# mrcdr/lambda-lanczos

Measured on AMD Instinct MI355X. Metric: Lanczos iterations/sec + SpMV GB/s (fp64, n=10M nnz=150M) at 1/2/4/8 GPUs, higher is better.
Workload: dtype f64; 1 GPU; random symmetric CSR n=10000000 nnz=150000000 fp64; n=10000000, nnz=150000000, partition=single GPU, orth_mode=0, tridiag_mode=2, eps=engine default

## Files before the change

### lambda-lanczos_amd/csrc/context.cpp

```cpp
#include <algorithm>
#include <cstdlib>
#include <memory>

#include "engine.hpp"

namespace ll {
static thread_local std::string g_last_error;
void set_error(const std::string& msg) { g_last_error = msg; }
}

using namespace ll;

namespace ll {
namespace {
long long to_ll(const std::string& v) { return std::atoll(v.c_str()); }
bool to_flag(const std::string& v) { return std::atoi(v.c_str()) != 0; }
int Tuning::*pauli_bits_key(const std::string& key) {
  static const std::pair<const char*, int Tuning::*> keys[] = {
      {"pauli_tile_bits", &Tuning::pauli_tile_bits}, {"pauli_sector_block_bits", &Tuning::pauli_sector_block_bits},
      {"pauli_momentum_block_bits", &Tuning::pauli_momentum_block_bits},
      {"pauli_momentum_full_block_bits", &Tuning::pauli_momentum_full_block_bits},
      {"pauli_symmetric_block_bits", &Tuning::pauli_symmetric_block_bits},
      {"pauli_rdm_tile_bits", &Tuning::pauli_rdm_tile_bits}, {"pauli_rdm_block_bits", &Tuning::pauli_rdm_block_bits}};
  for (const auto& k : keys)
// ... 17 lines not shown
  else if (key == "pair_gs") t.pair_gs = e ? d.pair_gs : to_flag(v);
  else if (key == "block_gs") t.block_gs = e ? d.block_gs : to_flag(v);
  else if (key == "pb_diag") t.pb_diag = e ? d.pb_diag : to_flag(v);
  else if (key == "fuse_launches") {
    const long long level = e ? 2 : to_ll(v);
    t.fuse_launches = level >= 1;
    t.lagged_gs = level >= 2;
  } else if (key == "blas_small_bytes") t.blas_small_bytes = e ? d.blas_small_bytes : to_ll(v);
  else if (key == "tridiag_thread") t.tridiag_thread = e ? d.tridiag_thread : to_flag(v);
  else if (key == "tridiag_lag") t.tridiag_lag = e ? d.tridiag_lag : (int)to_ll(v);
  else if (key == "dgks_threshold") t.dgks_threshold = e ? d.dgks_threshold : std::atof(v.c_str());
  else if (key == "slab_bytes") t.slab_bytes = e ? d.slab_bytes : std::max<long long>(1, to_ll(v));
  else if (key == "pb_block") t.pb_block = e ? 0 : (int)std::max<long long>(0, to_ll(v));
  else if (key == "pb_row_block") t.pb_row_block = e ? 0 : (int)std::max<long long>(0, to_ll(v));
  else if (key == "pb_col_block") t.pb_col_block = e ? 0 : (int)std::max<long long>(0, to_ll(v));
  else if (key == "pb_threads1") {
    t.pb_threads1 = e ? 0 : (int)to_ll(v);
    if (t.pb_threads1 != 256 && t.pb_threads1 != 512 && t.pb_threads1 != 1024) t.pb_threads1 = 0;
  } else if (key == "pb_pad") {
    t.pb_pad = e ? 0 : (int)to_ll(v);
    if (t.pb_pad != 4 && t.pb_pad != 16) t.pb_pad = 0;
  } else if (key == "pb_xpre") t.pb_xpre = e ? d.pb_xpre : to_flag(v);
  else if (key == "pb_test_all_remote") t.pb_test_all_remote = e ? false : to_flag(v);
  else if (key == "force_rp64") t.force_rp64 = e ? false : to_flag(v);
  else if (key == "spmv_tile_balance") t.spmv_tile_balance = e ? d.spmv_tile_balance : to_flag(v);
  else if (int Tuning::*bits = pauli_bits_key(key)) t.*bits = e ? d.*bits : (int)std::max<long long>(0, std::min<long long>(30, to_ll(v)));
  else if (key == "stencil_vec") t.stencil_vec = e ? d.stencil_vec : to_flag(v);
  else if (key == "tl_force") t.tl_force = e ? false : to_flag(v);
  else if (key == "tl_xcd") t.tl_xcd_order = e ? d.tl_xcd_order : to_flag(v);
  else if (key == "tl_walk") t.tl_walk_modulo = e ? d.tl_walk_modulo : to_flag(v);
  else if (key == "ritz_tail") t.ritz_tail = e ? d.ritz_tail : to_flag(v);
  else if (key == "event_in_launch") t.event_in_launch = e ? d.event_in_launch : to_flag(v);
  else if (key == "sweep_pipeline") t.sweep_pipeline = e ? d.sweep_pipeline : (int)std::max<long long>(0, std::min<long long>(2, to_ll(v)));
  else if (key == "pair_split") t.pair_split_vecs = e ? 0 : (int)std::max<long long>(0, to_ll(v));
  else if (key == "pair_max_stored") t.pair_max_stored = e ? 0 : (int)std::max<long long>(0, to_ll(v));
  else if (key == "lagged_pieces") t.lagged_pieces = e ? 0 : (int)to_ll(v);
  else if (key == "lagged_min_bytes") t.lagged_min_bytes = e ? -1 : to_ll(v);
  else if (key == "tridiag_test_jitter_us") t.tridiag_test_jitter_us = e ? 0 : (int)to_ll(v);
  else if (key == "test_workspace_fill") t.test_workspace_fill = e ? -1 : (int)std::max<long long>(0, std::min<long long>(255, to_ll(v)));
  else if (key == "stall_trace") t.stall_trace_ms = e ? -1.0 : std::atof(v.c_str());
  else return false;
  return true;
}
static const char* const kEnvSwitches[][2] = {
    {"LL_SPMV_KERNEL", "spmv_kernel"},       {"LL_SPMV_KEEP_BOTH", "spmv_keep_both"}, {"LL_PB_PHASE2", "pb_phase2"},
    {"LL_PB_PLACEMENTS", "pb_placements"},   {"LL_PB_PLACEMENT_TRACE", "pb_placement_trace"},
    {"LL_COMM_OVERLAP", "comm_overlap"},     {"LL_GATHER_CHUNKS", "gather_chunks"},   {"LL_CSR_SPLIT", "csr_split"},
    {"LL_ITER_TRACE", "iter_trace"},         {"LL_SHARDED_NORM", "sharded_norm"},     {"LL_PAIR_GS", "pair_gs"},
    {"LL_PB_DIAG", "pb_diag"},               {"LL_FUSE_LAUNCHES", "fuse_launches"},   {"LL_BLAS_SMALL_BYTES", "blas_small_bytes"},
    {"LL_TRIDIAG_THREAD", "tridiag_thread"}, {"LL_TRIDIAG_LAG", "tridiag_lag"},       {"LL_DGKS_THRESHOLD", "dgks_threshold"},
    {"LL_SLAB_BYTES", "slab_bytes"},
};
Tuning read_tuning(const std::map<std::string, std::string>* overrides) {
  Tuning t;
  for (auto& sw : kEnvSwitches) {
    const char* e = std::getenv(sw[0]);
    if (e && *e) (void)tuning_apply(t, sw[1], e);
  }
  if (overrides)
    for (auto& kv : *overrides) (void)tuning_apply(t, kv.first, kv.second);
  return t;
}
}

static size_t grow(size_t have, size_t want) { return std::max(want, have + have / 2 + 64); }

// ... 436 lines not shown
```

### lambda-lanczos_amd/csrc/gs_block.hip

```cpp
#include <algorithm>

#include "gs_strips.hpp"

namespace ll {

namespace {
__device__ __forceinline__ void block_sum2_all(double& a, double& b, double* sh) {
  a = wave_sum(a);
  b = wave_sum(b);
  const int lane = threadIdx.x & 63, wave = threadIdx.x >> 6;
  __syncthreads();
  if (lane == 0) {
    sh[wave] = a;
    sh[4 + wave] = b;
  }
  __syncthreads();
  a = (sh[0] + sh[1]) + (sh[2] + sh[3]);
  b = (sh[4] + sh[5]) + (sh[6] + sh[7]);
}
__device__ __forceinline__ void block_max2_all(double& a, double& b, double* sh) {
#pragma unroll
  for (int d = 32; d > 0; d >>= 1) {
    a = fmax(a, __shfl_down(a, d, 64));
    b = fmax(b, __shfl_down(b, d, 64));
// ... 4 lines not shown
    sh[wave] = a;
    sh[4 + wave] = b;
  }
  __syncthreads();
  a = fmax(fmax(sh[0], sh[1]), fmax(sh[2], sh[3]));
  b = fmax(fmax(sh[4], sh[5]), fmax(sh[6], sh[7]));
}
__device__ __forceinline__ double block_tri_row(const double* __restrict__ ha, const double* __restrict__ hb, const double* v, int i,
                                                int reals, int m, double alpha_last) {
  const int j = i / reals;
  double t = (j == m - 1 ? alpha_last : ha[j]) * v[i];
  if (j >= 1) t = fma(hb[j - 1], v[i - reals], t);
  if (j + 1 < m) t = fma(hb[j], v[i + reals], t);
  return t;
}
__device__ __forceinline__ size_t block_row_at(int reals, int j) { return (size_t)reals * (size_t)j * (size_t)(j - 1) / 2; }
}

__global__ __launch_bounds__(256) void block_enter_kernel(int k, int reals, const double* __restrict__ g, const double* __restrict__ c1,
                                                          double* __restrict__ rho2, double* __restrict__ cpk) {
  const int tid = threadIdx.x;
  for (int j = tid; j < k; j += 256) rho2[j] = 1.0;
  if (tid == 0) rho2[k] = *c1;
  double* rk1 = cpk + block_row_at(reals, k - 1);
  for (int i = tid; i < reals * (k - 1); i += 256) rk1[i] = 0.0;
  double* rk = cpk + block_row_at(reals, k);
  for (int i = tid; i < reals * k; i += 256) rk[i] = g[i];
}
void launch_block_enter(int k, int reals, const double* g, const double* c1, double* rho2, double* cpk, hipStream_t s) {
  hipLaunchKernelGGL(block_enter_kernel, dim3(1), dim3(256), 0, s, k, reals, g, c1, rho2, cpk);
  LL_HIP(hipGetLastError());
}

__global__ __launch_bounds__(256) void block_predict_kernel(int k, int m, int reals, BlockScalars sc, const double* __restrict__ rho2,
                                                            const double* __restrict__ cpk, double* __restrict__ hist_alpha,
                                                            const double* __restrict__ hist_beta, double* __restrict__ dk,
                                                            double* __restrict__ p, int pstride, double* __restrict__ prA,
                                                            double* __restrict__ prB) {
  __shared__ double red[8];
  const int tid = threadIdx.x;
  const int W = k + 1, RW = reals * W;
  const double* ck = cpk + block_row_at(reals, k);
  const double* ck1 = cpk + block_row_at(reals, k - 1);
  const double rk = sqrt(rho2[k]), rk1 = sqrt(rho2[k - 1]);
  const double ik = 1.0 / rk, ik1 = 1.0 / rk1;
  const double e0 = *sc.e[0];
  for (int i = tid; i < RW; i += 256) dk[i] = i < reals * k ? ck[i] * ik : 0.0;
  __syncthreads();
  double qa = 0.0, zero_ = 0.0;
  for (int i = tid; i < reals * k; i += 256) qa = fma(dk[i], block_tri_row(hist_alpha, hist_beta, dk, i, reals, k, hist_alpha[k - 1]), qa);
  block_sum2_all(qa, zero_, red);
  const double ake = -2.0 * ck[reals * (k - 1)] - qa;
  const double alpha_k = e0 + ake;
  if (tid == 0) hist_alpha[k] = alpha_k;
  for (int i = tid; i < RW; i += 256) {
    const double t = block_tri_row(hist_alpha, hist_beta, dk, i, reals, W, alpha_k);
    const double d1 = i < reals * (k - 1) ? ck1[i] * ik1 : 0.0;
    double v = t - e0 * dk[i] - rk * d1;
    if (i == reals * k) v += ake;
    p[i] = v;
  }
  __syncthreads();
  for (int s = 1; s < m; ++s) {
    const double* in = p + (size_t)(s - 1) * pstride;
    const double nin = sqrt(*sc.nsq[s - 1]), inv = 1.0 / nin;
    const double* prev = s == 1 ? dk : p + (size_t)(s - 2) * pstride;
    const double pinv = s == 1 ? 1.0 : 1.0 / sqrt(*sc.nsq[s - 2]);
    const double es = *sc.e[s];
    double* out = p + (size_t)s * pstride;
    for (int i = tid; i < RW; i += 256) {
      const double t = block_tri_row(hist_alpha, hist_beta, in, i, reals, W, alpha_k);
      out[i] = (t - es * in[i]) * inv - nin * (prev[i] * pinv);
    }
    __syncthreads();
  }
  for (int i = tid; i < RW; i += 256) {
    const double ir = 1.0 / sqrt(rho2[i / reals]);
    prA[i] = p[(size_t)(m - 1) * pstride + i] * ir;
    prB[i] = m >= 2 ? p[(size_t)(m - 2) * pstride + i] * ir : 0.0;
  }
}
void launch_block_predict(int k, int m, int reals, const BlockScalars& sc, const double* rho2, const double* cpk, double* hist_alpha,
                          const double* hist_beta, double* dk, double* p, int pstride, double* prA, double* prB, hipStream_t s) {
  hipLaunchKernelGGL(block_predict_kernel, dim3(1), dim3(256), 0, s, k, m, reals, sc, rho2, cpk, hist_alpha, hist_beta, dk, p, pstride, prA,
                     prB);
  LL_HIP(hipGetLastError());
}

template <typename T, int NV, int PC, int M>
__device__ __forceinline__ void block_trip_compute(const T (&ur)[NV][strip<T, PC>::EPT], int nv, const T (&b)[M][strip<T, PC>::EPT],
                                                   T (&cA)[strip<T, PC>::EPT], T (&cB)[strip<T, PC>::EPT],
                                                   const double* __restrict__ prAc, const double* __restrict__ prBc, double* mine,
                                                   int setstride, int lane) {
  constexpr int EPT = strip<T, PC>::EPT;
  double sre[M][NV], sim[M][NV];
#pragma unroll
  for (int v = 0; v < NV; ++v) {
    acc_t<T> ca, cb;
    const int vv = v < nv ? v : nv - 1;
    const bool real = v < nv;
    if constexpr (scalar_traits<T>::is_complex) {
      const double xa = ld_const(prAc, 2 * vv), ya = ld_const(prAc, 2 * vv + 1), xb = ld_const(prBc, 2 * vv), yb = ld_const(prBc, 2 * vv + 1);
      ca = zc{real ? xa : 0.0, real ? ya : 0.0};
      cb = zc{real ? xb : 0.0, real ? yb : 0.0};
    } else {
      const double xa = ld_const(prAc, vv), xb = ld_const(prBc, vv);
      ca = real ? xa : 0.0;
      cb = real ? xb : 0.0;
    }
    acc_t<T> sm[M];
#pragma unroll
    for (int i = 0; i < M; ++i) sm[i] = zero<acc_t<T>>();
#pragma unroll
    for (int e = 0; e < EPT; ++e) {
      fnma_acc(cA[e], ca, ur[v][e]);
      if constexpr (M >= 2) fnma_acc(cB[e], cb, ur[v][e]);
#pragma unroll
      for (int i = 0; i < M; ++i) cfma_acc(sm[i], ur[v][e], b[i][e]);
    }
#pragma unroll
    for (int i = 0; i < M; ++i) {
      if constexpr (scalar_traits<T>::is_complex) {
        sre[i][v] = sm[i].re;
        sim[i][v] = sm[i].im;
      } else {
        sre[i][v] = sm[i];
        sim[i][v] = 0.0;
      }
    }
  }
  constexpr int LPI = 64 / NV;
#pragma unroll
  for (int i = 0; i < M; ++i) {
    wave_sum_transposed<NV>(sre[i], lane);
    if constexpr (scalar_traits<T>::is_complex) wave_sum_transposed<NV>(sim[i], lane);
  }
  if ((lane & (LPI - 1)) == 0 && lane / LPI < nv) {
    const int v = lane / LPI;
#pragma unroll
    for (int i = 0; i < M; ++i) {
      if constexpr (scalar_traits<T>::is_complex) {
        mine[i * setstride + 2 * v] += sre[i][0];
        mine[i * setstride + 2 * v + 1] += sim[i][0];
      } else {
        mine[i * setstride + v] += sre[i][0];
      }
    }
  }
}

template <typename T, int PC, int M, int JB>
__global__ __launch_bounds__(kBlock) void block_sweep_kernel(int64_t n, const T* const* __restrict__ vtab, int W, int col0, int Wl, int flags,
                                                             BlockVecs<T> bv, const double* __restrict__ prA,
                                                             const double* __restrict__ prB, double* __restrict__ partials) {
  constexpr int EPT = strip<T, PC>::EPT;
  constexpr int ELEMS = strip<T, PC>::ELEMS;
  constexpr int R = scalar_traits<T>::reals;
  constexpr int NG = R * M * (M - 1) / 2 + M;
  const bool first = (flags & kPairFirst) != 0, last = (flags & kPairLast) != 0;
  const int ncols = M * R * W + NG;
  const int lcols = M * R * Wl + (last ? NG : 0);
  extern __shared__ double lds[];
  const int tid = threadIdx.x, lane = tid & 63, wave = tid >> 6;
  for (int i = tid; i < 4 * lcols; i += kBlock) lds[i] = 0.0;
  __syncthreads();
  double* mine = lds + (size_t)wave * lcols;
  double* tail = mine + M * R * Wl;
  const T* const* tab = vtab + col0;
  const double *prAc = prA + R * col0, *prBc = prB + R * col0;
  const int ntrips = (Wl + JB - 1) / JB;
  const int64_t nstrips = (n + ELEMS - 1) / ELEMS;
  T* const outA = last ? bv.b[M - 1] : bv.part[0];
  T* const outB = last ? bv.b[M >= 2 ? M - 2 : 0] : bv.part[1];

  auto do_strip = [&](auto full_c, const int64_t base) {
    constexpr bool FULL = decltype(full_c)::value;
    T b[M][EPT], cA[EPT], cB[EPT];
#pragma unroll
    for (int i = 0; i < M; ++i) load_lstrip_u<T, PC, FULL>(bv.b[i], base, n, b[i]);
    auto issue = [&](T (&buf)[JB][EPT], int t) {
      const T* ptr[JB];
#pragma unroll
      for (int v = 0; v < JB; ++v) ptr[v] = ld_const_ptr<T>(tab, min(JB * t + v, Wl - 1));
#pragma unroll
      for (int v = 0; v < JB; ++v) load_lstrip_u<T, PC, FULL>(ptr[v], base, n, buf[v]);
    };
    T ua[JB][EPT], ub[JB][EPT];
    if (ntrips > 0) {
      __builtin_amdgcn_sched_barrier(0);
      issue(ua, 0);
      __builtin_amdgcn_sched_barrier(0);
    }
    if (first) {
#pragma unroll
      for (int e = 0; e < EPT; ++e) {
        cA[e] = b[M - 1][e];
        cB[e] = b[M >= 2 ? M - 2 : 0][e];
      }
    } else {
      load_lstrip_u<T, PC, FULL>(bv.part[0], base, n, cA);
      if constexpr (M >= 2) load_lstrip_u<T, PC, FULL>(bv.part[1], base, n, cB);
    }
    for (int t = 0; t < ntrips; t += 2) {
      __builtin_amdgcn_sched_barrier(0);
      issue(ub, t + 1);
      __builtin_amdgcn_sched_barrier(0);
      block_trip_compute<T, JB, PC, M>(ua, min(JB, Wl - JB * t), b, cA, cB, prAc + R * JB * t, prBc + R * JB * t, mine + R * JB * t, R * Wl, lane);
      if (t + 1 >= ntrips) break;
      __builtin_amdgcn_sched_barrier(0);
      issue(ua, t + 2);
      __builtin_amdgcn_sched_barrier(0);
      block_trip_compute<T, JB, PC, M>(ub, min(JB, Wl - JB * (t + 1)), b, cA, cB, prAc + R * JB * (t + 1), prBc + R * JB * (t + 1),
                                       mine + R * JB * (t + 1), R * Wl, lane);
    }
    store_lstrip_u<T, PC, FULL>(outA, base, n, cA);
    if constexpr (M >= 2) store_lstrip_u<T, PC, FULL>(outB, base, n, cB);
    if (!last) return;
#pragma unroll
    for (int e = 0; e < EPT; ++e) {
      b[M - 1][e] = cA[e];
      if constexpr (M >= 2) b[M - 2][e] = cB[e];
    }
    int at = 0;
#pragma unroll
    for (int i = 1; i < M; ++i) {
#pragma unroll
      for (int ip = 0; ip < i; ++ip) {
        acc_t<T> g = zero<acc_t<T>>();
#pragma unroll
        for (int e = 0; e < EPT; ++e) cfma_acc(g, b[ip][e], b[i][e]);
        const acc_t<T> gs = wave_sum(g);
        if (lane == 0) {
          if constexpr (scalar_traits<T>::is_complex) {
            tail[at] += gs.re;
            tail[at + 1] += gs.im;
          } else {
            tail[at] += gs;
          }
        }
        at += R;
      }
    }
#pragma unroll
    for (int i = 0; i < M; ++i) {
      double nn = 0.0;
#pragma unroll
      for (int e = 0; e < EPT; ++e) nn += abs2(b[i][e]);
      nn = wave_sum(nn);
      if (lane == 0) tail[at + i] += nn;
    }
  };
  for (int64_t sidx = blockIdx.x; sidx < nstrips; sidx += gridDim.x) {
    const int64_t base = sidx * ELEMS;
    if (base + ELEMS <= n) do_strip(std::true_type{}, base);
    else do_strip(std::false_type{}, base);
  }
  __syncthreads();
  double* out = partials + (size_t)blockIdx.x * ncols;
  for (int i = tid; i < lcols; i += kBlock) {
    const double v = (lds[i] + lds[lcols + i]) + (lds[2 * lcols + i] + lds[3 * lcols + i]);
    int g;
    if (i < M * R * Wl) {
      const int set = i / (R * Wl);
      g = set * R * W + R * col0 + (i - set * R * Wl);
    } else {
      g = M * R * W + (i - M * R * Wl);
    }
    out[g] = v;
  }
}
constexpr int kBlockJB = 2;
template <typename T, int PC, int M>
static void block_sweep_launch(int grid, size_t lds_bytes, hipStream_t s, int64_t n, const T* const* vtab, int W, int col0, int Wl, int flags,
                               const BlockVecs<T>& bv, const double* prA, const double* prB, double* partials) {
  hipLaunchKernelGGL((block_sweep_kernel<T, PC, M, kBlockJB>), dim3(grid), dim3(kBlock), lds_bytes, s, n, vtab, W, col0, Wl, flags, bv, prA, prB,
                     partials);
}
template <typename T>
int launch_block_sweep(int64_t n, const T* const* vtab, int W, int m, const BlockVecs<T>& bv, const double* prA, const double* prB,
                       double* partials, int pieces, int per_launch, hipStream_t s) {
  constexpr int R = scalar_traits<T>::reals;
  LL_REQUIRE(m == 1 || m == 2 || m == 4, "internal: block sweep of 1, 2 or 4 iterations");
  const int64_t strips16k = (n * (int64_t)sizeof(T) + 16383) / 16384;
  int pc = strips16k >= kLaggedFullStrips ? 4 : 2;
  if (pieces == 2 || pieces == 4) pc = pieces;
  const int grid = pc == 4 ? strip_grid(n, strip<T, 4>::ELEMS) : strip_grid(n, strip<T, 2>::ELEMS);
  const int ng = R * m * (m - 1) / 2 + m;
  per_launch = std::max(1, std::min(per_launch, block_sweep_max_vecs<T>(m)));
  for (int col0 = 0; col0 < W; col0 += per_launch) {
    const int Wl = std::min(per_launch, W - col0);
    const int flags = (col0 == 0 ? kPairFirst : 0) | (col0 + Wl == W ? kPairLast : 0);
    const size_t lds_bytes = (size_t)4 * (size_t)(m * R * Wl + ((flags & kPairLast) ? ng : 0)) * sizeof(double);
#define LL_BLOCK_SWEEP(PC_, M_) block_sweep_launch<T, PC_, M_>(grid, lds_bytes, s, n, vtab, W, col0, Wl, flags, bv, prA, prB, partials)
    if (pc == 4) {
      if (m == 4) LL_BLOCK_SWEEP(4, 4);
      else if (m == 2) LL_BLOCK_SWEEP(4, 2);
      else LL_BLOCK_SWEEP(4, 1);
    } else {
      if (m == 4) LL_BLOCK_SWEEP(2, 4);
      else if (m == 2) LL_BLOCK_SWEEP(2, 2);
      else LL_BLOCK_SWEEP(2, 1);
    }
#undef LL_BLOCK_SWEEP
    LL_HIP(hipGetLastError());
  }
  return grid;
}

__global__ __launch_bounds__(256) void block_fold_kernel(const double* __restrict__ cols, int k, int m, int reals, BlockScalars sc,
                                                         const double* __restrict__ p, int pstride, double* __restrict__ rho2,
                                                         double* __restrict__ cpk, double* __restrict__ hist_alpha,
                                                         double* __restrict__ hist_beta, double* __restrict__ raw0,
                                                         double* __restrict__ raw1, BlockHost host) {
  __shared__ double red[8];
  const int tid = threadIdx.x;
  const int W = k + 1, RW = reals * W;
  const double* tail = cols + (size_t)m * RW;
  const double* diag = tail + reals * m * (m - 1) / 2;
  for (int s = 0; s < m; ++s) {
    const int j = k + 1 + s;
    double* raw = (s & 1) ? raw1 : raw0;
    const double* rawp = (s & 1) ? raw0 : raw1;
    double* row = cpk + block_row_at(reals, j);
    const double* ms = cols + (size_t)s * RW;
    const double* ps = p + (size_t)s * pstride;
    const bool comp = s == m - 1 || s == m - 2;
    const double nn = diag[s], nraw2 = *sc.nsq[s];
    for (int i = tid; i < RW; i += 256) raw[i] = ms[i] / sqrt(rho2[i / reals]);
    __syncthreads();
    for (int col = k - 1; col <= k; ++col) {
      const double* cr = cpk + block_row_at(reals, col);
      double dre = 0.0, dim = 0.0;
      for (int l = tid; l < col; l += 256) {
        if (reals == 2) {
          const double ar = cr[2 * l], ai = cr[2 * l + 1], br = raw[2 * l], bi = raw[2 * l + 1];
          dre += ar * br + ai * bi;
          dim += ar * bi - ai * br;
        } else {
          dre += cr[l] * raw[l];
        }
      }
      block_sum2_all(dre, dim, red);
      if (tid == 0) {
        const double ir = 1.0 / sqrt(rho2[col]);
        raw[reals * col] = (ms[reals * col] - dre) * ir;
        if (reals == 2) raw[2 * col + 1] = (ms[2 * col + 1] - dim) * ir;
      }
      __syncthreads();
    }
    double mxr = 0.0, mxc = 0.0, cc = 0.0;
    for (int i = tid; i < RW; i += 256) {
      const double v = comp ? raw[i] - ps[i] : raw[i];
      row[i] = v;
      mxr = fmax(mxr, fabs(raw[i]));
      mxc = fmax(mxc, fabs(v));
      cc = fma(v, v, cc);
    }
    __syncthreads();
    for (int sp = 0; sp < s; ++sp) {
      const int col = k + 1 + sp;
// ... 28 lines not shown
    }
    double zero_ = 0.0;
    block_sum2_all(cc, zero_, red);
    block_max2_all(mxr, mxc, red);
    double r2 = nn - cc;
    r2 = r2 > 0.0 ? r2 : 0.0;
    double alpha_pub;
    if (s == 0) {
      alpha_pub = hist_alpha[k];
    } else {
      double qb = 0.0;
      for (int i = tid; i < reals * (j - 1); i += 256)
        qb = fma(rawp[i], block_tri_row(hist_alpha, hist_beta, rawp, i, reals, j - 1, hist_alpha[j - 2]), qb);
      block_sum2_all(qb, zero_, red);
      const double rp2 = rho2[j - 1];
      alpha_pub = rp2 > 0.0 ? (*sc.e[s] * *sc.nsq[s - 1] - 2.0 * rp2 * rawp[reals * (j - 2)] - qb) / rp2 : 0.0;
    }
    __syncthreads();
    if (tid == 0) {
      rho2[j] = r2;
      hist_beta[j - 1] = sqrt(r2);
      if (s > 0) hist_alpha[j - 1] = alpha_pub;
      double gate = 1.0;
      if (nn > 0.0 && nraw2 > 0.0) gate = fmax(mxr / sqrt(nraw2), mxc / sqrt(nn));
      host.slot[s][0] = alpha_pub;
      host.slot[s][1] = r2;
      host.slot[s][2] = nn;
      host.slot[s][3] = r2;
      *host.gate[s] = gate;
    }
    __syncthreads();
  }
}
void launch_block_fold(const double* cols, int k, int m, int reals, const BlockScalars& sc, const double* p, int pstride, double* rho2,
                       double* cpk, double* hist_alpha, double* hist_beta, double* raw0, double* raw1, const BlockHost& host, hipStream_t s,
                       hipEvent_t stop) {
  LL_LAUNCH_STOP(stop, block_fold_kernel, dim3(1), dim3(256), 0, s, cols, k, m, reals, sc, p, pstride, rho2, cpk, hist_alpha, hist_beta, raw0,
                 raw1, host);
  LL_HIP(hipGetLastError());
}

template int launch_block_sweep<double>(int64_t, const double* const*, int, int, const BlockVecs<double>&, const double*, const double*,
                                        double*, int, int, hipStream_t);
template int launch_block_sweep<zc>(int64_t, const zc* const*, int, int, const BlockVecs<zc>&, const double*, const double*, double*, int, int,
                                    hipStream_t);

}
```

### lambda-lanczos_amd/csrc/lanczos_loop.hpp

```cpp
#pragma once

#include "engine.hpp"
#include "loop_support.hpp"
#include "raw_basis.hpp"
#include "ritz_tracker.hpp"
#include "trace.hpp"

#include <algorithm>
#include <cmath>
#include <limits>
#include <string>
#include <variant>

namespace ll {


template <typename T> struct LoopState {
  Engine<T>& E;
  Basis<T>& U;
  EventRing& ring;
  PhaseTimer& timer;
  int64_t nl;
  hipStream_t s;
  bool fuse_launches = true, defer = false;
// ... 382 lines not shown
    coeff = pair_coeff_over_raw(R, g1h, g2h, std::sqrt(rho[0]), std::sqrt(rho[1]), n_locked, Pt, tail.nvec, m, nw, coeff);
    basis = basis_runs(Pt);
    basis.add(tail.pair.r[0], 1);
    if (tail.nvec == 2) basis.add(tail.pair.r[1], 1);
    return basis;
  }
  int64_t enqueue_block(int64_t kk, double offset) {
    if constexpr (sizeof(typename scalar_traits<T>::real) == 8) return enqueue_block_f64(kk, offset);
    else return 0;
  }
  int64_t enqueue_block_f64(int64_t kk, double offset) {
    constexpr int R = Engine<T>::R;
    const Tuning& tune = E.ctx->tune;
    if (!block_enabled || !block_allowed || !pair_allowed || !lag_ok || n_locked != 0) return 0;
    const BlockIter* const bi = pending_as<BlockIter>();
    const LaggedIter* const lg = pending_as<LaggedIter>();
    int64_t k;
    if (bi) {
      if (bi->k + 1 != kk) return 0;
      k = bi->k;
    } else if (lg && lg->k == kk - 1 && kk >= 3) {
      k = kk - 1;
    } else {
      return 0;
    }
    const int64_t remaining = max_k_hint - (kk - 1);
    if (remaining < 1) return 0;
    const int m = remaining >= 4 ? 4 : (remaining >= 2 ? 2 : 1);
    const int64_t strips16k = (nl * (int64_t)sizeof(T) + 16383) / 16384;
    const bool streaming = tune.sweep_pipeline >= 2 || strips16k > 2 * kCUs + kCUs / 4;
    if (!streaming || vec_bytes() < stream_bytes() || k + m + 1 > bb.cap || (size_t)(k + m + 1) > kVtabCap) return 0;
    if (tune.pair_max_stored > 0 && k + 1 > tune.pair_max_stored) return 0;
    const int W = (int)(k + 1);
    const int ncols = m * R * W + R * m * (m - 1) / 2 + m;
    int per_launch = block_sweep_max_vecs<T>(m);
    if (tune.pair_split_vecs > 0) per_launch = std::min(per_launch, std::max(1, tune.pair_split_vecs));
    if (W > per_launch)
      for (auto& b : bsplit)
        if (!b.p) b.alloc(E.ctx, (size_t)ld);
    const double te0 = now_s();
    want_partial_cols((size_t)std::max(ncols, 1 + R));
    if (!bi) {
      LL_HIP(hipMemcpyAsync(U.vec(k), work[k & 1].p, (size_t)nl * sizeof(T), hipMemcpyDeviceToDevice, s));
      launch_block_enter((int)k, R, lb.g[k & 1], lg->c1, bb.rho2, bb.cpk, s);
      blk_k0 = k;
    }
    BlockVecs<T> bv{};
    for (int i = 0; i < m; ++i) bv.b[i] = U.vec(k + 1 + i);
    bv.part[0] = bsplit[0].p;
    bv.part[1] = bsplit[1].p;
    const T* const* vt = vtab_sync();
    BlockScalars sc{};
    BlockHost host{};
    int slots[4] = {0, 0, 0, 0};
    for (int i = 0; i < 4; ++i) {
      const int ii = std::min(i, m - 1);
      slots[i] = (int)((kk + ii) % kRingSlots);
      sc.e[i] = E.S(kScalAlpha + slots[i]);
      sc.nsq[i] = bb.nsq + 4 * ii;
      host.slot[i] = pinned_slot(slots[i]);
      host.gate[i] = pinned_gate(slots[i]);
    }
    for (int i = 0; i < m; ++i) {
      const T* x = i == 0 ? U.vec(k) : bv.b[i - 1];
      const T* xp = i == 0 ? U.vec(k - 1) : (i == 1 ? U.vec(k) : bv.b[i - 2]);
      const double* xn2 = i == 0 ? bb.rho2 + k : bb.nsq + 4 * (i - 1);
      const double* pn2 = i == 0 ? bb.rho2 + k - 1 : (i == 1 ? bb.rho2 + k : bb.nsq + 4 * (i - 2));
      double* e = E.S(kScalAlpha + slots[i]);
      timer.mark();
      typename Engine<T>::DeferredAlpha da;
      E.apply(x, bv.b[i], offset, e, true, fuse_launches ? &da : nullptr, nullptr, xn2);
      timer.mark();
      const int g3 = launch_pair_three_term<T>(nl, bv.b[i], x, xp, e, da.nparts > 0 ? da.partials : nullptr, da.nparts, xn2, pn2,
                                               E.ctx->partials.get(), false, s);
      launch_reduce_cols(E.ctx->partials.get(), g3, 1 + R, bb.nsq + 4 * i, nullptr, s);
      if (i + 1 < m) timer.mark();
    }
    launch_block_predict((int)k, m, R, sc, bb.rho2, bb.cpk, lb.hist_alpha, lb.hist_beta, bb.dk, bb.p, (int)bb.rec, bb.prA, bb.prB, s);
    const int grid = launch_block_sweep<T>(nl, vt, W, m, bv, bb.prA, bb.prB, E.ctx->partials.get(), tune.lagged_pieces, per_launch, s);
    launch_reduce_cols(E.ctx->partials.get(), grid, ncols, bb.cols, nullptr, s);
    const int ev = slots[m - 1];
    launch_block_fold(bb.cols, (int)k, m, R, sc, bb.p, (int)bb.rec, bb.rho2, bb.cpk, lb.hist_alpha, lb.hist_beta, bb.raw0, bb.raw1, host, s,
                      tune.event_in_launch ? ring.ev[ev] : nullptr);
    if (!tune.event_in_launch) LL_HIP(hipEventRecord(ring.ev[ev], s));
    timer.mark();
    for (int i = 0; i < m; ++i) {
      ev_of_slot[slots[i]] = ev;
      slot_pair[slots[i]] = true;
    }
    pending = BlockIter{k + m};
    n_block += m;
    if (m >= 2) n_pair += m;
    n_lagged += m;
    t_enqueue += now_s() - te0;
    return m;
  }
  bool enqueue_pair(int64_t k, double offset) {
    constexpr int R = Engine<T>::R;
    if (!pair_enabled || !pair_allowed || !lag_ok) return false;
    if (max_k_hint > 0 && k + 1 > max_k_hint) return false;
    const int64_t Lk = n_locked;
    PairIter in;
    if (const PairIter* pr = pending_as<PairIter>()) {
      if (pr->P + 2 != k) return false;
      in = *pr;
    } else if (const LaggedIter* lg = pending_as<LaggedIter>(); lg && lg->k == k - 1 && k >= 3) {
      in = PairIter{k - 2, {U.vec(k - 2), work[(k - 1) & 1].p}, {pb.zero, lb.g[(k - 1) & 1]}, {pb.scal + 0, lg->c1}, 0, 1};
    } else {
      return false;
    }
    const int64_t P = in.P;
    const T *const r1 = in.r[0], *const r2 = in.r[1];
    const double *const g1 = in.g[0], *const g2 = in.g[1], *const rho1sq = in.rho2[0], *const rho2sq = in.rho2[1];
    const int out_set = in.set ^ 1, out_rec = in.rec ^ 1;
    const int64_t K = Lk + P;
// ... 354 lines not shown
```

### lambda-lanczos_amd/csrc/ll_internal.hpp

```cpp
#pragma once

#include <hip/hip_runtime.h>
#if defined(__HIPCC__)
#include <hip/hip_ext.h>
#endif

#include <algorithm>
#include <atomic>
#include <cstdint>
#include <cstdio>
#include <cstring>
#include <map>
#include <memory>
#include <string>
#include <type_traits>
#include <vector>

#include "../../include/lanczos_hip.h"
#include "../../include/lanczos_hip_transport.h"
#include "scalar_types.hpp"
#include "spmv_plan.hpp"

#if defined(__HIPCC__)
#define LL_LAUNCH_STOP(stop, kernel, grid, block, lds, s, ...)                                      \
// ... 151 lines not shown
namespace ll {
struct Tuning {
  int spmv_kernel = -1;
  bool keep_both = false;
  int pb_phase2 = 4;
  int pb_block = 0;
  int pb_row_block = 0;
  int pb_col_block = 0;
  int pair_max_stored = 0;
  int pair_split_vecs = 0;
  int pb_threads1 = 0;
  int pb_pad = 0;
  int pb_placements = 8;
  bool pb_xpre = true;
  bool pb_diag = true;
  int gather_chunks = 0;
  bool spmv_tile_balance = true;
  bool csr_split = true;
  bool comm_overlap = true;
  bool tridiag_thread = true;
  int tridiag_lag = 3;
  double dgks_threshold = 0.5;
  bool sharded_norm_measured = false;
  int64_t slab_bytes = (int64_t)4 << 30;
  int64_t blas_small_bytes = (int64_t)4 << 20;
  bool fuse_launches = true;
  long long lagged_min_bytes = -1;
  int lagged_pieces = 0;
  bool lagged_gs = true;
  bool event_in_launch = true;
  bool ritz_tail = true;
  int sweep_pipeline = 1;
  bool block_gs = true;
  bool pair_gs = true;
  bool force_rp64 = false;
  bool tl_xcd_order = true;
  bool tl_walk_modulo = true;
  bool tl_force = false;
  bool pb_test_all_remote = false;
  int tridiag_test_jitter_us = 0;
  int pauli_tile_bits = -1;
  int pauli_momentum_block_bits = -1;
  int pauli_momentum_full_block_bits = -1;
  int pauli_symmetric_block_bits = -1;
  int pauli_sector_block_bits = -1;
  int pauli_rdm_tile_bits = -1;
  int pauli_rdm_block_bits = -1;
  int test_workspace_fill = -1;
  bool stencil_vec = true;
  double stall_trace_ms = -1.0;
  std::string iter_trace;
  bool pb_placement_trace = false;
};
Tuning read_tuning(const std::map<std::string, std::string>* overrides);
bool tuning_apply(Tuning& t, const std::string& key, const std::string& value);

}

struct ll_context {
  ll::Tuning tune;
  std::map<std::string, std::string> tuning_overrides;
  int device = 0;
  hipStream_t stream = nullptr;
  bool own_stream = false;
  ll::Comm* comm = nullptr;
  int rank = 0, nranks = 1;
// ... 427 lines not shown
template <typename T> constexpr int pair_sweep_max_vecs() {
  return (kLaggedMaxCols - 5 * scalar_traits<T>::reals - 1) / (2 * scalar_traits<T>::reals);
}
template <typename T>
int launch_pair_sweep(int64_t n, const std::vector<BasisSegs<T>>& groups, int P, const T* r1, const T* r2, const T* r3, T* r4,
                      T* uP_out, T* uQ_out, T* part4, const double* g1, const double* g2, const double* gam, const double* p4,
                      const double* rho1sq, const double* rho2sq, const double* e2, const double* n3sq, double* partials, int pieces,
                      hipStream_t s, const T* const* vtab = nullptr,
                      bool force_pipeline = false);
template <typename T>
bool launch_pair_sweep_small(int64_t n, const BasisSegs<T>& segs, int P, const T* r1, const T* r2, const T* r3, T* r4, T* uP_out,
                             T* uQ_out, const double* g1, const double* g2, const double* gam, const double* p4, const double* rho1sq,
                             const double* rho2sq, const double* e2, const double* n3sq, double* partials, int* grid_out,
                             hipStream_t s);
template <typename T> bool pair_small_fits(int P);
template <typename T> void launch_fill_ptrs(const T** tab, int start, int count, const T* base, int64_t ld, hipStream_t s);
void launch_pair_fold(const double* m, int P, int L, int reals, const double* lambda, const double* p4, const double* g2, const double* gam,
                      const double* rho2sq, const double* n3sq, const double* e1, const double* e2, double* rec3, double* rec4,
                      double* nxt, double* hist_alpha, double* hist_beta, double* scratch, double* host_a, double* host_b,
                      double* gate_a, double* gate_b, hipStream_t s, hipEvent_t stop = nullptr);
constexpr int kBlockMaxVecs = 1024;
struct BlockScalars {
  const double* e[4];
  const double* nsq[4];
};
struct BlockHost {
  double* slot[4];
  double* gate[4];
};
template <typename T> struct BlockVecs {
  T* b[4];
  T* part[2];
};
template <typename T> constexpr int block_sweep_max_vecs(int m) {
  return (kLaggedMaxCols - (scalar_traits<T>::reals * m * (m - 1) / 2 + m)) / (m * scalar_traits<T>::reals);
}
void launch_block_enter(int k, int reals, const double* g, const double* c1, double* rho2, double* cpk, hipStream_t s);
void launch_block_predict(int k, int m, int reals, const BlockScalars& sc, const double* rho2, const double* cpk, double* hist_alpha,
                          const double* hist_beta, double* dk, double* p, int pstride, double* prA, double* prB, hipStream_t s);
template <typename T>
int launch_block_sweep(int64_t n, const T* const* vtab, int W, int m, const BlockVecs<T>& bv, const double* prA, const double* prB,
                       double* partials, int pieces, int per_launch, hipStream_t s);
void launch_block_fold(const double* cols, int k, int m, int reals, const BlockScalars& sc, const double* p, int pstride, double* rho2,
                       double* cpk, double* hist_alpha, double* hist_beta, double* raw0, double* raw1, const BlockHost& host, hipStream_t s,
                       hipEvent_t stop = nullptr);
void launch_lagged_fold(double* m, int K, int L, int reals, double* t_out, const double* c0, double* c0_out, double* c1,
                        double* alpha, const double* prev_g, const double* prev_t, const double* prev_c1,
                        double* hist_alpha, double* hist_beta, const double* lambda, double* host_mapped, hipStream_t s, hipEvent_t stop = nullptr);
template <typename T>
int launch_maxpy(int64_t n, T* w, const BasisSegs<T>& segs, const double* h, const NormRefs* pred, double* partials,
                 int64_t small_bytes, hipStream_t s);
template <typename T>
bool launch_maxpy_folding(int64_t n, T* w, const BasisSegs<T>& segs, const double* mdot_partials, int mparts, double* h_out,
                          double* c0_out, double* partials, int64_t small_bytes, int* grid_out, hipStream_t s);
template <typename T> void launch_scale(int64_t n, T* v, double a, const NormRefs* norms, hipStream_t s);
template <typename T>
void launch_scale_derive(int64_t n, T* v, const double* c0_src, const double* h, int count, double* c0, double* c1,
                         const double* alpha, double* host_mapped, hipStream_t s);
template <typename T>
int launch_scale_publish(int64_t n, T* v, const double* partials, int nparts, double* out, const double* alpha,
                         const double* c0, double* host_mapped, hipStream_t s, const T* src = nullptr);
template <typename T>
void launch_three_term(int64_t n, T* w, const T* u_prev, const T* u_cur, double beta, double alpha, hipStream_t s);
constexpr int kRecurRec = 4;
template <typename T>
int launch_recur_step(int64_t n, T* y, const T* x, const T* p, const double* alpha_partials, int alpha_nparts, double* rec,
                      int64_t k, bool normalised, double* partials, hipStream_t s);
void launch_recur_fold(const double* partials, int nparts, double* rec, int64_t k, double* host_mapped, hipStream_t s);
template <typename T>
void launch_recur_accum(int64_t n, T* y, const T* x, const T* p, T* psi, const double* rec, const double* gvec, int64_t k,
                        double a, double b, double g, const double* alpha_partials, int alpha_nparts, long long* mismatches,
                        hipStream_t s);
template <typename T>
void launch_recur_accum_cplx(int64_t n, T* y, const T* x, const T* p, T* psi, const double* rec, const zc* gvec, int64_t k,
                             double a, double b, zc g, const double* alpha_partials, int alpha_nparts, long long* mismatches,
                             hipStream_t s);
constexpr int kRecurMultiMax = 16;
constexpr int kRecurMultiBatch = 2;
// ... 33 lines not shown
```

Before: 874.4 Lanczos iterations/s.

## Fuse the block's last three-term update and norm into the block GS sweep

```diff
diff --git a/lambda-lanczos_amd/csrc/context.cpp b/lambda-lanczos_amd/csrc/context.cpp
--- a/lambda-lanczos_amd/csrc/context.cpp
+++ b/lambda-lanczos_amd/csrc/context.cpp
@@ -73,6 +73,7 @@
   else if (key == "ritz_tail") t.ritz_tail = e ? d.ritz_tail : to_flag(v);
   else if (key == "event_in_launch") t.event_in_launch = e ? d.event_in_launch : to_flag(v);
   else if (key == "sweep_pipeline") t.sweep_pipeline = e ? d.sweep_pipeline : (int)std::max<long long>(0, std::min<long long>(2, to_ll(v)));
+  else if (key == "block_last_in_sweep") t.block_last_in_sweep = e ? d.block_last_in_sweep : to_flag(v);
   else if (key == "pair_split") t.pair_split_vecs = e ? 0 : (int)std::max<long long>(0, to_ll(v));
   else if (key == "pair_max_stored") t.pair_max_stored = e ? 0 : (int)std::max<long long>(0, to_ll(v));
   else if (key == "lagged_pieces") t.lagged_pieces = e ? 0 : (int)to_ll(v);
diff --git a/lambda-lanczos_amd/csrc/gs_block.hip b/lambda-lanczos_amd/csrc/gs_block.hip
--- a/lambda-lanczos_amd/csrc/gs_block.hip
+++ b/lambda-lanczos_amd/csrc/gs_block.hip
@@ -60,19 +60,26 @@
   LL_HIP(hipGetLastError());
 }
 
-__global__ __launch_bounds__(256) void block_predict_kernel(int k, int m, int reals, BlockScalars sc, const double* __restrict__ rho2,
+__global__ __launch_bounds__(256) void block_predict_kernel(int k, int m, int reals, BlockScalars sc, const double* __restrict__ e_partials,
+                                                            int e_nparts, double* __restrict__ e_out, const double* __restrict__ rho2,
                                                             const double* __restrict__ cpk, double* __restrict__ hist_alpha,
                                                             const double* __restrict__ hist_beta, double* __restrict__ dk,
                                                             double* __restrict__ p, int pstride, double* __restrict__ prA,
                                                             double* __restrict__ prB) {
   __shared__ double red[8];
   const int tid = threadIdx.x;
+  double e_last = 0.0;
+  if (e_partials) {
+    e_last = fold_partials_all(e_partials, e_nparts, red);
+    if (tid == 0) *e_out = e_last;
+    __syncthreads();
+  }
   const int W = k + 1, RW = reals * W;
   const double* ck = cpk + block_row_at(reals, k);
   const double* ck1 = cpk + block_row_at(reals, k - 1);
   const double rk = sqrt(rho2[k]), rk1 = sqrt(rho2[k - 1]);
   const double ik = 1.0 / rk, ik1 = 1.0 / rk1;
-  const double e0 = *sc.e[0];
+  const double e0 = (e_partials && m == 1) ? e_last : *sc.e[0];
   for (int i = tid; i < RW; i += 256) dk[i] = i < reals * k ? ck[i] * ik : 0.0;
   __syncthreads();
   double qa = 0.0, zero_ = 0.0;
@@ -94,7 +101,7 @@
     const double nin = sqrt(*sc.nsq[s - 1]), inv = 1.0 / nin;
     const double* prev = s == 1 ? dk : p + (size_t)(s - 2) * pstride;
     const double pinv = s == 1 ? 1.0 : 1.0 / sqrt(*sc.nsq[s - 2]);
-    const double es = *sc.e[s];
+    const double es = (e_partials && s == m - 1) ? e_last : *sc.e[s];
     double* out = p + (size_t)s * pstride;
     for (int i = tid; i < RW; i += 256) {
       const double t = block_tri_row(hist_alpha, hist_beta, in, i, reals, W, alpha_k);
@@ -108,10 +115,11 @@
     prB[i] = m >= 2 ? p[(size_t)(m - 2) * pstride + i] * ir : 0.0;
   }
 }
-void launch_block_predict(int k, int m, int reals, const BlockScalars& sc, const double* rho2, const double* cpk, double* hist_alpha,
-                          const double* hist_beta, double* dk, double* p, int pstride, double* prA, double* prB, hipStream_t s) {
-  hipLaunchKernelGGL(block_predict_kernel, dim3(1), dim3(256), 0, s, k, m, reals, sc, rho2, cpk, hist_alpha, hist_beta, dk, p, pstride, prA,
-                     prB);
+void launch_block_predict(int k, int m, int reals, const BlockScalars& sc, const BlockLastScalars& last, const double* rho2,
+                          const double* cpk, double* hist_alpha, const double* hist_beta, double* dk, double* p, int pstride, double* prA,
+                          double* prB, hipStream_t s) {
+  hipLaunchKernelGGL(block_predict_kernel, dim3(1), dim3(256), 0, s, k, m, reals, sc, last.e ? last.e_partials : nullptr, last.e_nparts,
+                     last.e_out, rho2, cpk, hist_alpha, hist_beta, dk, p, pstride, prA, prB);
   LL_HIP(hipGetLastError());
 }
 
@@ -177,15 +185,31 @@
   }
 }
 
-template <typename T, int PC, int M, int JB>
+template <typename T> struct BlockLastArgs {
+  const T* x;
+  const T* p;
+  const double* e;
+  const double* cx2;
+  const double* cp2;
+};
+template <typename T, int PC, int M, int JB, bool L3>
 __global__ __launch_bounds__(kBlock) void block_sweep_kernel(int64_t n, const T* const* __restrict__ vtab, int W, int col0, int Wl, int flags,
                                                              BlockVecs<T> bv, const double* __restrict__ prA,
-                                                             const double* __restrict__ prB, double* __restrict__ partials) {
+                                                             const double* __restrict__ prB, double* __restrict__ partials,
+                                                             BlockLastArgs<T> lx) {
   constexpr int EPT = strip<T, PC>::EPT;
   constexpr int ELEMS = strip<T, PC>::ELEMS;
   constexpr int R = scalar_traits<T>::reals;
-  constexpr int NG = R * M * (M - 1) / 2 + M;
+  constexpr int NG = R * M * (M - 1) / 2 + M + (L3 ? 1 : 0);
   const bool first = (flags & kPairFirst) != 0, last = (flags & kPairLast) != 0;
+  double ca = 0.0, cb = 0.0;
+  if constexpr (L3) {
+    if (first) {
+      const double nx = sqrt(*lx.cx2);
+      ca = *lx.e / nx;
+      cb = nx / sqrt(*lx.cp2);
+    }
+  }
   const int ncols = M * R * W + NG;
   const int lcols = M * R * Wl + (last ? NG : 0);
   extern __shared__ double lds[];
@@ -220,6 +244,18 @@
       __builtin_amdgcn_sched_barrier(0);
     }
     if (first) {
+      if constexpr (L3) {
+        T xo[EPT], po[EPT];
+        if constexpr (M == 1) load_lstrip_u<T, PC, FULL>(lx.x, base, n, xo);
+        if constexpr (M <= 2) load_lstrip_u<T, PC, FULL>(lx.p, base, n, po);
+#pragma unroll
+        for (int e = 0; e < EPT; ++e) {
+          const T xe = M >= 2 ? b[M >= 2 ? M - 2 : 0][e] : xo[e];
+          const T pe = M >= 3 ? b[M >= 3 ? M - 3 : 0][e] : po[e];
+          b[M - 1][e] = sub(sub(b[M - 1][e], rmul(ca, xe)), rmul(cb, pe));
+        }
+        if (!last) store_lstrip_u<T, PC, FULL>(bv.b[M - 1], base, n, b[M - 1]);
+      }
 #pragma unroll
       for (int e = 0; e < EPT; ++e) {
         cA[e] = b[M - 1][e];
@@ -244,6 +280,13 @@
     store_lstrip_u<T, PC, FULL>(outA, base, n, cA);
     if constexpr (M >= 2) store_lstrip_u<T, PC, FULL>(outB, base, n, cB);
     if (!last) return;
+    if constexpr (L3) {
+      double nr = 0.0;
+#pragma unroll
+      for (int e = 0; e < EPT; ++e) nr += abs2(b[M - 1][e]);
+      nr = wave_sum(nr);
+      if (lane == 0) tail[NG - 1] += nr;
+    }
 #pragma unroll
     for (int e = 0; e < EPT; ++e) {
       b[M - 1][e] = cA[e];
@@ -298,28 +341,34 @@
   }
 }
 constexpr int kBlockJB = 2;
-template <typename T, int PC, int M>
+template <typename T, int PC, int M, bool L3>
 static void block_sweep_launch(int grid, size_t lds_bytes, hipStream_t s, int64_t n, const T* const* vtab, int W, int col0, int Wl, int flags,
-                               const BlockVecs<T>& bv, const double* prA, const double* prB, double* partials) {
-  hipLaunchKernelGGL((block_sweep_kernel<T, PC, M, kBlockJB>), dim3(grid), dim3(kBlock), lds_bytes, s, n, vtab, W, col0, Wl, flags, bv, prA, prB,
-                     partials);
+                               const BlockVecs<T>& bv, const double* prA, const double* prB, double* partials, const BlockLastArgs<T>& lx) {
+  hipLaunchKernelGGL((block_sweep_kernel<T, PC, M, kBlockJB, L3>), dim3(grid), dim3(kBlock), lds_bytes, s, n, vtab, W, col0, Wl, flags, bv, prA,
+                     prB, partials, lx);
 }
 template <typename T>
 int launch_block_sweep(int64_t n, const T* const* vtab, int W, int m, const BlockVecs<T>& bv, const double* prA, const double* prB,
-                       double* partials, int pieces, int per_launch, hipStream_t s) {
+                       double* partials, int pieces, int per_launch, const BlockLastScalars& last, const T* last_x, const T* last_p,
+                       hipStream_t s) {
   constexpr int R = scalar_traits<T>::reals;
   LL_REQUIRE(m == 1 || m == 2 || m == 4, "internal: block sweep of 1, 2 or 4 iterations");
   const int64_t strips16k = (n * (int64_t)sizeof(T) + 16383) / 16384;
   int pc = strips16k >= kLaggedFullStrips ? 4 : 2;
   if (pieces == 2 || pieces == 4) pc = pieces;
   const int grid = pc == 4 ? strip_grid(n, strip<T, 4>::ELEMS) : strip_grid(n, strip<T, 2>::ELEMS);
-  const int ng = R * m * (m - 1) / 2 + m;
-  per_launch = std::max(1, std::min(per_launch, block_sweep_max_vecs<T>(m)));
+  const bool l3 = last.e != nullptr;
+  LL_REQUIRE(!l3 || (last.cx2 && last.cp2 && (m >= 2 || last_x) && (m >= 3 || last_p)), "internal: operands of the block's last update");
+  const BlockLastArgs<T> lx{last_x, last_p, last.e, last.cx2, last.cp2};
+  const int ng = R * m * (m - 1) / 2 + m + (l3 ? 1 : 0);
+  per_launch = std::max(1, std::min(per_launch, block_sweep_max_vecs<T>(m, l3)));
   for (int col0 = 0; col0 < W; col0 += per_launch) {
     const int Wl = std::min(per_launch, W - col0);
     const int flags = (col0 == 0 ? kPairFirst : 0) | (col0 + Wl == W ? kPairLast : 0);
     const size_t lds_bytes = (size_t)4 * (size_t)(m * R * Wl + ((flags & kPairLast) ? ng : 0)) * sizeof(double);
-#define LL_BLOCK_SWEEP(PC_, M_) block_sweep_launch<T, PC_, M_>(grid, lds_bytes, s, n, vtab, W, col0, Wl, flags, bv, prA, prB, partials)
+#define LL_BLOCK_SWEEP(PC_, M_)                                                                                                     \
+  (l3 ? block_sweep_launch<T, PC_, M_, true>(grid, lds_bytes, s, n, vtab, W, col0, Wl, flags, bv, prA, prB, partials, lx)             \
+      : block_sweep_launch<T, PC_, M_, false>(grid, lds_bytes, s, n, vtab, W, col0, Wl, flags, bv, prA, prB, partials, lx))
     if (pc == 4) {
       if (m == 4) LL_BLOCK_SWEEP(4, 4);
       else if (m == 2) LL_BLOCK_SWEEP(4, 2);
@@ -336,6 +385,7 @@
 }
 
 __global__ __launch_bounds__(256) void block_fold_kernel(const double* __restrict__ cols, int k, int m, int reals, BlockScalars sc,
+                                                         int last_in_sweep,
                                                          const double* __restrict__ p, int pstride, double* __restrict__ rho2,
                                                          double* __restrict__ cpk, double* __restrict__ hist_alpha,
                                                          double* __restrict__ hist_beta, double* __restrict__ raw0,
@@ -353,7 +403,7 @@
     const double* ms = cols + (size_t)s * RW;
     const double* ps = p + (size_t)s * pstride;
     const bool comp = s == m - 1 || s == m - 2;
-    const double nn = diag[s], nraw2 = *sc.nsq[s];
+    const double nn = diag[s], nraw2 = (last_in_sweep && s == m - 1) ? diag[m] : *sc.nsq[s];
     for (int i = tid; i < RW; i += 256) raw[i] = ms[i] / sqrt(rho2[i / reals]);
     __syncthreads();
     for (int col = k - 1; col <= k; ++col) {
@@ -448,17 +498,17 @@
     __syncthreads();
   }
 }
-void launch_block_fold(const double* cols, int k, int m, int reals, const BlockScalars& sc, const double* p, int pstride, double* rho2,
-                       double* cpk, double* hist_alpha, double* hist_beta, double* raw0, double* raw1, const BlockHost& host, hipStream_t s,
-                       hipEvent_t stop) {
-  LL_LAUNCH_STOP(stop, block_fold_kernel, dim3(1), dim3(256), 0, s, cols, k, m, reals, sc, p, pstride, rho2, cpk, hist_alpha, hist_beta, raw0,
+void launch_block_fold(const double* cols, int k, int m, int reals, const BlockScalars& sc, bool last_in_sweep, const double* p, int pstride,
+                       double* rho2, double* cpk, double* hist_alpha, double* hist_beta, double* raw0, double* raw1, const BlockHost& host,
+                       hipStream_t s, hipEvent_t stop) {
+  LL_LAUNCH_STOP(stop, block_fold_kernel, dim3(1), dim3(256), 0, s, cols, k, m, reals, sc, last_in_sweep ? 1 : 0, p, pstride, rho2, cpk, hist_alpha, hist_beta, raw0,
                  raw1, host);
   LL_HIP(hipGetLastError());
 }
 
 template int launch_block_sweep<double>(int64_t, const double* const*, int, int, const BlockVecs<double>&, const double*, const double*,
-                                        double*, int, int, hipStream_t);
+                                        double*, int, int, const BlockLastScalars&, const double*, const double*, hipStream_t);
 template int launch_block_sweep<zc>(int64_t, const zc* const*, int, int, const BlockVecs<zc>&, const double*, const double*, double*, int, int,
-                                    hipStream_t);
-
-}
+                                    const BlockLastScalars&, const zc*, const zc*, hipStream_t);
+
+}
diff --git a/lambda-lanczos_amd/csrc/lanczos_loop.hpp b/lambda-lanczos_amd/csrc/lanczos_loop.hpp
--- a/lambda-lanczos_amd/csrc/lanczos_loop.hpp
+++ b/lambda-lanczos_amd/csrc/lanczos_loop.hpp
@@ -438,8 +438,9 @@
     if (!streaming || vec_bytes() < stream_bytes() || k + m + 1 > bb.cap || (size_t)(k + m + 1) > kVtabCap) return 0;
     if (tune.pair_max_stored > 0 && k + 1 > tune.pair_max_stored) return 0;
     const int W = (int)(k + 1);
-    const int ncols = m * R * W + R * m * (m - 1) / 2 + m;
-    int per_launch = block_sweep_max_vecs<T>(m);
+    const bool l3 = tune.block_last_in_sweep;
+    const int ncols = m * R * W + R * m * (m - 1) / 2 + m + (l3 ? 1 : 0);
+    int per_launch = block_sweep_max_vecs<T>(m, l3);
     if (tune.pair_split_vecs > 0) per_launch = std::min(per_launch, std::max(1, tune.pair_split_vecs));
     if (W > per_launch)
       for (auto& b : bsplit)
@@ -467,6 +468,8 @@
       host.slot[i] = pinned_slot(slots[i]);
       host.gate[i] = pinned_gate(slots[i]);
     }
+    BlockLastScalars last{};
+    const T *last_x = nullptr, *last_p = nullptr;
     for (int i = 0; i < m; ++i) {
       const T* x = i == 0 ? U.vec(k) : bv.b[i - 1];
       const T* xp = i == 0 ? U.vec(k - 1) : (i == 1 ? U.vec(k) : bv.b[i - 2]);
@@ -477,16 +480,23 @@
       typename Engine<T>::DeferredAlpha da;
       E.apply(x, bv.b[i], offset, e, true, fuse_launches ? &da : nullptr, nullptr, xn2);
       timer.mark();
+      if (l3 && i == m - 1) {
+        last = BlockLastScalars{e, xn2, pn2, da.nparts > 0 ? da.partials : nullptr, da.nparts, e};
+        last_x = x;
+        last_p = xp;
+        break;
+      }
       const int g3 = launch_pair_three_term<T>(nl, bv.b[i], x, xp, e, da.nparts > 0 ? da.partials : nullptr, da.nparts, xn2, pn2,
                                                E.ctx->partials.get(), false, s);
       launch_reduce_cols(E.ctx->partials.get(), g3, 1 + R, bb.nsq + 4 * i, nullptr, s);
       if (i + 1 < m) timer.mark();
     }
-    launch_block_predict((int)k, m, R, sc, bb.rho2, bb.cpk, lb.hist_alpha, lb.hist_beta, bb.dk, bb.p, (int)bb.rec, bb.prA, bb.prB, s);
-    const int grid = launch_block_sweep<T>(nl, vt, W, m, bv, bb.prA, bb.prB, E.ctx->partials.get(), tune.lagged_pieces, per_launch, s);
+    launch_block_predict((int)k, m, R, sc, last, bb.rho2, bb.cpk, lb.hist_alpha, lb.hist_beta, bb.dk, bb.p, (int)bb.rec, bb.prA, bb.prB, s);
+    const int grid = launch_block_sweep<T>(nl, vt, W, m, bv, bb.prA, bb.prB, E.ctx->partials.get(), tune.lagged_pieces, per_launch, last,
+                                            last_x, last_p, s);
     launch_reduce_cols(E.ctx->partials.get(), grid, ncols, bb.cols, nullptr, s);
     const int ev = slots[m - 1];
-    launch_block_fold(bb.cols, (int)k, m, R, sc, bb.p, (int)bb.rec, bb.rho2, bb.cpk, lb.hist_alpha, lb.hist_beta, bb.raw0, bb.raw1, host, s,
+    launch_block_fold(bb.cols, (int)k, m, R, sc, l3, bb.p, (int)bb.rec, bb.rho2, bb.cpk, lb.hist_alpha, lb.hist_beta, bb.raw0, bb.raw1, host, s,
                       tune.event_in_launch ? ring.ev[ev] : nullptr);
     if (!tune.event_in_launch) LL_HIP(hipEventRecord(ring.ev[ev], s));
     timer.mark();
diff --git a/lambda-lanczos_amd/csrc/ll_internal.hpp b/lambda-lanczos_amd/csrc/ll_internal.hpp
--- a/lambda-lanczos_amd/csrc/ll_internal.hpp
+++ b/lambda-lanczos_amd/csrc/ll_internal.hpp
@@ -207,6 +207,7 @@
   bool ritz_tail = true;
   int sweep_pipeline = 1;
   bool block_gs = true;
+  bool block_last_in_sweep = true;
   bool pair_gs = true;
   bool force_rp64 = false;
   bool tl_xcd_order = true;
@@ -700,18 +701,28 @@
   T* b[4];
   T* part[2];
 };
-template <typename T> constexpr int block_sweep_max_vecs(int m) {
-  return (kLaggedMaxCols - (scalar_traits<T>::reals * m * (m - 1) / 2 + m)) / (m * scalar_traits<T>::reals);
+struct BlockLastScalars {
+  const double* e = nullptr;
+  const double* cx2 = nullptr;
+  const double* cp2 = nullptr;
+  const double* e_partials = nullptr;
+  int e_nparts = 0;
+  double* e_out = nullptr;
+};
+template <typename T> constexpr int block_sweep_max_vecs(int m, bool last_in_sweep = false) {
+  return (kLaggedMaxCols - (scalar_traits<T>::reals * m * (m - 1) / 2 + m + (last_in_sweep ? 1 : 0))) / (m * scalar_traits<T>::reals);
 }
 void launch_block_enter(int k, int reals, const double* g, const double* c1, double* rho2, double* cpk, hipStream_t s);
-void launch_block_predict(int k, int m, int reals, const BlockScalars& sc, const double* rho2, const double* cpk, double* hist_alpha,
-                          const double* hist_beta, double* dk, double* p, int pstride, double* prA, double* prB, hipStream_t s);
+void launch_block_predict(int k, int m, int reals, const BlockScalars& sc, const BlockLastScalars& last, const double* rho2,
+                          const double* cpk, double* hist_alpha, const double* hist_beta, double* dk, double* p, int pstride, double* prA,
+                          double* prB, hipStream_t s);
 template <typename T>
 int launch_block_sweep(int64_t n, const T* const* vtab, int W, int m, const BlockVecs<T>& bv, const double* prA, const double* prB,
-                       double* partials, int pieces, int per_launch, hipStream_t s);
-void launch_block_fold(const double* cols, int k, int m, int reals, const BlockScalars& sc, const double* p, int pstride, double* rho2,
-                       double* cpk, double* hist_alpha, double* hist_beta, double* raw0, double* raw1, const BlockHost& host, hipStream_t s,
-                       hipEvent_t stop = nullptr);
+                       double* partials, int pieces, int per_launch, const BlockLastScalars& last, const T* last_x, const T* last_p,
+                       hipStream_t s);
+void launch_block_fold(const double* cols, int k, int m, int reals, const BlockScalars& sc, bool last_in_sweep, const double* p, int pstride,
+                       double* rho2, double* cpk, double* hist_alpha, double* hist_beta, double* raw0, double* raw1, const BlockHost& host,
+                       hipStream_t s, hipEvent_t stop = nullptr);
 void launch_lagged_fold(double* m, int K, int L, int reals, double* t_out, const double* c0, double* c0_out, double* c1,
                         double* alpha, const double* prev_g, const double* prev_t, const double* prev_c1,
                         double* hist_alpha, double* hist_beta, const double* lambda, double* host_mapped, hipStream_t s, hipEvent_t stop = nullptr);
```

New measurement: 888.0 Lanczos iterations/s (median of 6 runs). +1.6%, better.
